# EmreAdabag/osqp

Hardware: AMD Instinct MI355X
Metric: ADMM iters/sec (single QP) (higher is better)
Workload: dtype f64; 1 GPU; config2 random sparse QP n=10000 m=20000 nnzA=200000 nnzPtriu=59985, one step = osqp_update_rho(0.1) + cold-started osqp_solve; adaptive_rho_interval=100, status=solved, graph_launches=4775, resident_gave_up=0, resident_slow_waits=0, parallelism=replicas x1 (a single QP does not shard)

## Files before the change

include/osqp_amd_engine.h:

```cpp
#ifndef OSQP_AMD_ENGINE_H
#define OSQP_AMD_ENGINE_H

#include "osqp_amd_types.h"

#ifdef __cplusplus
extern "C" {
#endif

#define HIPENG_OK            0
#define HIPENG_ERR_NO_DEVICE (-101)
#define HIPENG_ERR_HIP       (-102)
#define HIPENG_ERR_ARG       (-103)
#define HIPENG_ERR_ALLOC     (-104)

typedef struct hipeng hipeng;

typedef struct {
  c_float sigma;
  c_float alpha;
  c_float pcg_eps_rel;
  c_float pcg_eps_abs;
  c_int   pcg_max_iter;
  c_int   no_restart;
} hipeng_params;
// ... 50 lines not shown
int hipeng_certificates(hipeng *e, c_float eps_dx, int unscaled, hipeng_scalars *inout);
int hipeng_download(hipeng *e, c_float *x, c_float *y, c_float *z, c_float *dx,
                    c_float *dy, int dy_projected);
int hipeng_get_stats(hipeng *e, hipeng_stats *st);
int hipeng_reset_stats(hipeng *e);
int hipeng_sync(hipeng *e);

int hipeng_kkt_solve(hipeng *e, c_float *b);
int hipeng_kkt_solve_unrefined(hipeng *e, c_float *b);

int hipeng_spmv(hipeng *e, int which, const c_float *x, c_float *y);
int hipeng_spmv_dev(hipeng *e, int which, const c_float *d_x, c_float *d_y);
int hipeng_time_kernel(hipeng *e, int which, int reps, double *usec);
int hipeng_kernel_bytes(hipeng *e, int which, double *bytes);
int hipeng_is_split(hipeng *e);
int hipeng_pcg_layout(hipeng *e, long long out[16]);
int hipeng_row_eliminated(hipeng *e, c_int i);
c_int hipeng_elim_count(hipeng *e);
int hipeng_elim_peek(hipeng *e, int which, c_float *out);
int hipeng_resident_info(hipeng *e, long long out[16]);
int hipeng_resident_trips(hipeng *e, long long out[8]);
int hipeng_resident_plan(const csc *P, const csc *A, int nwg, long long stats[8], int *Kptr, int *Kcol, int *kdst, long long cap,
                         unsigned short *rowpos, unsigned short *slotcol, int *wg4);
long long hipeng_resident_plan_lists(const csc *P, const csc *A, int nwg, int *Kcp, int *Kcm, int *Kca, long long cap);
int hipeng_form_k_info(hipeng *e, long long out[4]);
long long hipeng_resident_dump(hipeng *e, int *row, int *col, double *val, long long cap);

int hipeng_dense_invert_selftest(int n, const double *A, double *Ainv, double *ms);
int hipeng_dense_invert_route(int n, const double *A, double *Ainv, int route, int gemm);
int hipeng_dense_switches(int out[2]);
int hipeng_dense_gemm_selftest(int kernel, int M, int N, int K, const double *T, int ldt, const double *B, int ldb, const double *w,
                               double *C, int ldc, double alpha, double beta, int sr0, int sr1, int sc0, int sc1, int lower, int kmode, int ksl);

int hipeng_switch_row(int index, const char **name, int *kind, char *def_text, int def_cap, int *unset_distinct, const char **what);
int hipeng_switch_values(double *out, int rows);

typedef struct hipsens hipsens;
int hipsens_create(hipsens **out, c_int n, c_int m, c_int nnzP, c_int nnzA, int device);
void hipsens_destroy(hipsens *s);
int hipsens_set_point(hipsens *s, hipeng *pe, const c_float *x, const c_float *yact, const c_int *act,
                      const c_float *D, const c_float *E, c_float c);
int hipsens_grad(hipsens *s, hipeng *pe, const csc *P, const csc *A, const c_float *rx, const c_float *rnu,
                 c_float *dPx, c_float *dAx);
int hipsens_tan_rhs(hipsens *s, hipeng *pe, const csc *P, const csc *A, c_int ndir, const c_float *dq, const c_float *dl,
                    const c_float *du, const c_float *dPx, const c_float *dAx, c_float *g);

// ... 15 lines not shown
```

osqp_amd/csrc/engine.hip:

```cpp
#include <hip/hip_runtime.h>
#include <cstdio>
#include <new>
#include <cstdlib>
#include <cstring>
#include <cstddef>
#include <climits>
#include <limits>
#include <cmath>
#include <vector>
#include <map>
#include <algorithm>
#include <mutex>
#include <condition_variable>
#include <thread>
#include <atomic>
#include <chrono>
#include "../../include/osqp_amd_engine.h"

#define TB 256
#define MAX_CHUNK 2048
#define LONG_ROW 512
#define HUGE_ROW 8192
#define MAX_PARTS 1024
#define MAX_HUGE_FOLD 4
// ... 1017 lines not shown
    __syncthreads();
  }
  for (int bi = c.A.nwave + blockIdx.x; bi < c.A.nblk; bi += gridDim.x) {
    const double zt = huge_row_sum(c, bi, red);
    if (threadIdx.x == 0) row_update(c.A.blk[bi].r0, zt);
    __syncthreads();
  }
  TLK_AT(8, 0); TLK_LAST(1);
  TLK_FLUSH(c, 110, 9);
}


#define RES_TB 512
#define RES_PT (RES_TB - 64)
#define RES_MAXROWS 61
#define RES_MAXN (RES_MAXROWS * 256)
#define RES_MAXPAD 16384
#define RES_MAXLD (RES_MAXPAD / 2 / RES_TB)
#define RES_WAIT_TICKS 2000000LL
#define RES_SLOW_TICKS 5000LL
#define AUX_SC1 16
#define AUX_VOL ((int)0x80000000)
#define RES_DBG 16
#define RES_PRED_WINDOW 16
#define RES_FSTRIDE 32
#define RES_GSTRIDE 16
typedef unsigned int u32x4 __attribute__((ext_vector_type(4)));
typedef unsigned int u32x2 __attribute__((ext_vector_type(2)));
struct ResWG { int r0, nr, cnt, pos; };
struct ResCtx {
  int nwg, E, npad;
  int npw;
  const unsigned short *rowpos;
  int pipe;
  int predict;
  double pred_margin;
  int u0_direct;
  int inject;
  const ResWG *wg;
  const int *ppos;
  double *val;
  const unsigned short *col;
  const unsigned char *rowl;
  const int *krp, *kcj, *kps, *kdst;
  const unsigned long long *brk;
  const unsigned short *slot0;
  const unsigned short *segrow;
  double *ubuf;
  unsigned *flags;
  int *dbg;
  double *sbuf;
  double *r0pos;
  const int *kcp, *kcm, *kca;
};

static __device__ __forceinline__ __amdgpu_buffer_rsrc_t res_rsrc(const void *p, size_t bytes) {
  return __builtin_amdgcn_make_buffer_rsrc(const_cast<void *>(p), 0, (int)bytes, 0x00020000);
}

__device__ __forceinline__ int res_spin_check(State *st, long long &t0, int &late) {
// ... 147 lines not shown
      }
#pragma unroll
      for (int q = 0; q < 4; ++q)
        if (eb + q * 64 + lane < e1) {
          const bool gone = c.nelim && (igone || c.erow[j[q]] >= 0);
          rc.val[dst[q]] = gone ? (j[q] == i ? 1.0 : 0.0) : v[q];
        }
    }
  }
}

template <int E>
__global__ void __launch_bounds__(RES_TB) k_pcg_resident(Ctx c, ResCtx rc) {
  extern __shared__ __attribute__((aligned(16))) double rlds[];
  State *st = c.st;
  TL_MARK(c, 5);
  const int s_stalled = st->stalled, s_run = st->run, s_fail = st->res_fail;
  const unsigned ep0 = st->res_epoch;
  const int s_pipe_off = st->res_pipe_off, s_pred_off = st->res_pred_off, s_admm_done = st->admm_done;
  const Params prm = *c.prm;
  const ResWG w = rc.wg[blockIdx.x];
  if ((s_stalled != 0) | (s_run == 0) | (s_fail != 0)) return;
  double *uv = rlds;
  double *seg = uv + rc.npad;
  double *sc = seg + RES_TB + RES_MAXROWS;
  double *sval = sc + 8;
#ifdef OSQP_AMD_TIMELINE
  long long *tls = reinterpret_cast<long long *>(sval + 768);
#define RTL(k) do { if (blockIdx.x == 0 && threadIdx.x == 0 && nx >= 1 && nx <= 64) tls[(nx - 1) * 5 + (k)] = wall_clock64(); } while (0)
  long long *wtl = tls + 5 * 64;
#define WTL(k) do { if (blockIdx.x == 0 && (threadIdx.x & 63) == 0 && (nx == 8 || nx == 1)) wtl[(nx == 1 ? 40 : 0) + (k) * 8 + (threadIdx.x >> 6)] = wall_clock64(); } while (0)
  if (blockIdx.x == 0 && threadIdx.x == 0) wtl[80] = wall_clock64();
#else
#define RTL(k) do { } while (0)
#define WTL(k) do { } while (0)
#endif
  const int g = blockIdx.x, t = threadIdx.x, lane = t & 63, wv = t >> 6;
  const int nwg = rc.nwg, npad = rc.npad;
  const bool sabotage = rc.inject > 0 && g == rc.nwg - 1 && s_admm_done + 1 == rc.inject;
  bool pipe = rc.pipe && !s_pipe_off && !prm.no_restart;
  bool predict = pipe && rc.predict && !s_pred_off;
  const bool prod = wv != 0;
  const int tt = t - 64;
  double kv[E]; unsigned short kc[E];
#pragma unroll
  for (int k = 0; k < E; ++k) { kv[k] = 0.0; kc[k] = 0; }
  unsigned long long brk = 0ull;
  int slot0 = 0;
  const bool u0_direct = rc.u0_direct != 0;
  u32x4 u0v[RES_MAXLD];
  auto u0_issue = [&]() __attribute__((always_inline)) {
    const __amdgpu_buffer_rsrc_t ru = res_rsrc(c.u0pos, (size_t)npad * 8);
#pragma unroll
    for (int q = 0; q < RES_MAXLD; ++q) u0v[q] = __builtin_amdgcn_raw_buffer_load_b128(ru, (q * RES_TB + t) * 16, 0, 0);
  };
  if (prod) {
    if (u0_direct) u0_issue();
#pragma unroll
    for (int k = 0; k < E; ++k) {
      const size_t idx = ((size_t)g * E + k) * RES_PT + tt;
      kv[k] = rc.val[idx]; kc[k] = rc.col[idx];
    }
    brk = rc.brk[(size_t)g * RES_PT + tt];
    slot0 = rc.slot0[(size_t)g * RES_PT + tt];
  }
  int sr0 = 0, sr1 = 0;
  int ppos[4] = {0, 0, 0, 0};
  constexpr int NPL = MAX_PARTS / 64;
  static_assert(NPL == 16 && NPL * 64 == MAX_PARTS, "k_pcg_resident: a lane of wavefront 0 holds MAX_PARTS / 64 partials of each start-up sum");
  double own_r = 0.0, own_u = 0.0, own_x = 0.0, own_mi = 0.0;
  if (!prod) {
    const int gm = c.gridM;
    double pr[NPL], pb[NPL];
#pragma unroll
    for (int q = 0; q < NPL; ++q) { const int i = min(lane + 64 * q, gm - 1); pr[q] = c.part_rr[i]; pb[q] = c.part_bb[i]; }
#pragma unroll
    for (int q = 0; q < 4; ++q) ppos[q] = rc.ppos[min(lane + 64 * q, nwg - 1)];
    const int jc = min(w.r0 + lane, c.n - 1), pc = min(w.pos + lane, npad - 1);
    const bool rpos = rc.r0pos != nullptr;
    const double *rsrc = rpos ? rc.r0pos : c.init_r, *usrc = rpos ? c.u0pos : c.init_z;
    own_r = rsrc[rpos ? (size_t)pc : (size_t)jc * c.init_stride]; own_u = usrc[rpos ? pc : jc]; own_x = c.vx[jc]; own_mi = c.minv[jc];
    sr0 = rc.segrow[(size_t)g * (RES_MAXROWS + 1) + min(lane, RES_MAXROWS)]; sr1 = rc.segrow[(size_t)g * (RES_MAXROWS + 1) + min(lane + 1, RES_MAXROWS)];
    double rr0 = 0.0, bb = 0.0;
#pragma unroll
    for (int q = 0; q < NPL; ++q) { const bool in = lane + 64 * q < gm; rr0 += in ? pr[q] : 0.0; bb += in ? pb[q] : 0.0; }
    rr0 = wave_sum(rr0); bb = wave_sum(bb);
    const double tl2 = fmax(prm.eps_rel * prm.eps_rel * bb, prm.eps_abs * prm.eps_abs);
    if (lane == 0) { sc[3] = 0.0; sc[5] = tl2; sc[6] = rr0 <= tl2 ? 1.0 : 0.0; }
    if (u0_direct) u0_issue();
  }
  const bool own = wv == 0 && lane < w.nr;
  const int j = w.r0 + lane;
  double rs_rest[11] = {0, 0, 0, 0, 0, 0, 0, 0, 0, 0, 0};
#define RES_ROWSTATE(i) (*((i) < E ? &kv[(i) < E ? (i) : 0] : &rs_rest[i]))
  double &r_ = RES_ROWSTATE(0), &u_ = RES_ROWSTATE(1), &w_ = RES_ROWSTATE(2), &p_ = RES_ROWSTATE(3), &s_ = RES_ROWSTATE(4), &x_ = RES_ROWSTATE(5);
  double &mi = RES_ROWSTATE(6), &x0_ = RES_ROWSTATE(7), &r0_ = RES_ROWSTATE(8);
  double &z_ = RES_ROWSTATE(9), &q_ = RES_ROWSTATE(10);
#undef RES_ROWSTATE
  if (own) { r_ = own_r; u_ = own_u; x_ = own_x; mi = own_mi; x0_ = own_x; r0_ = own_r; }
  else { sr0 = 0; sr1 = 0; }
  if (u0_direct) {
    const int half = npad >> 1;
#pragma unroll
    for (int q = 0; q < RES_MAXLD; ++q) {
      const int i2 = q * RES_TB + t;
      if (i2 < half) { uv[2 * i2] = __hiloint2double((int)u0v[q].y, (int)u0v[q].x); uv[2 * i2 + 1] = __hiloint2double((int)u0v[q].w, (int)u0v[q].z); }
    }
  }
  __syncthreads();
  const double tol2 = sc[5];
  if (sc[6] != 0.0) {
    if (g == 0 && t == 0) { st->done = 1; st->tol2 = tol2; }
    return;
  }
  int nx = 0;
  unsigned tag = ep0;
  int par = 0;

  auto vec_exchange = [&](double val, bool ride) __attribute__((always_inline)) -> bool {
    double e0 = 0.0, e1 = 0.0, e2 = 0.0;
    ++nx; tag = ep0 + (unsigned)nx; par = (int)(tag & 1u);
    if (sabotage && nx == 3) return false;
    RTL(0);
    const __amdgpu_buffer_rsrc_t rs = res_rsrc(rc.ubuf + (size_t)par * npad, (size_t)npad * 8);
    if (wv == 0) {
      if (lane < w.nr) {
        u32x2 d; d.x = (unsigned)__double2loint(val); d.y = (unsigned)__double2hiint(val);
        __builtin_amdgcn_raw_buffer_store_b64(d, rs, (w.pos + lane) * 8, 0, AUX_SC1);
      }
      if (ride) { e0 = wave_sum(own ? r_ * u_ : 0.0); e1 = wave_sum(own ? w_ * u_ : 0.0); e2 = wave_sum(own ? r_ * r_ : 0.0); }
      if (lane < 3) {
        const double v = lane == 0 ? e0 : (lane == 1 ? e1 : e2);
        u32x2 d; d.x = (unsigned)__double2loint(v); d.y = (unsigned)__double2hiint(v);
        __builtin_amdgcn_raw_buffer_store_b64(d, rs, (w.pos + w.nr + lane) * 8, 0, AUX_SC1);
      }
      asm volatile("s_waitcnt vmcnt(0)" ::: "memory");
      if (lane == 0) __hip_atomic_store(rc.flags + (size_t)g * RES_FSTRIDE, tag, __ATOMIC_RELAXED, __HIP_MEMORY_SCOPE_AGENT);
    }
    if (wv < rc.npw) {
      const int o = t;
// ... 14 lines not shown
        if (verdict) {
          const unsigned long long miss = __ballot(pend);
          const int fl = miss ? (int)__ffsll((long long)miss) - 1 : 0;
          const unsigned sv = (unsigned)__builtin_amdgcn_readlane((int)seen, fl);
          if (lane == 0) { res_note(st, rc.dbg, g, verdict, 1, nx, miss ? 64 * wv + fl : -1, sv, t0, rounds, 0); sc[3] = 1.0; }
          gave = true;
          break;
        }
        if (rounds == 16u) { const unsigned long long ms = __ballot(pend); miss16 = ms ? 64 * wv + (int)__ffsll((long long)ms) - 1 : -1; }
        if ((rounds & 63u) == 0 && wv == 0 && lane == 0) {
          __hip_atomic_store(rc.flags + (size_t)g * RES_FSTRIDE, tag, __ATOMIC_RELAXED, __HIP_MEMORY_SCOPE_AGENT);
          atomicAdd(&st->res_repub, 1);
        }
        if ((rounds & 255u) == 0) __builtin_amdgcn_fence(__ATOMIC_ACQUIRE, "agent");
        __builtin_amdgcn_s_sleep(1);
      }
      if (rounds >= 16u && lane == 0 && !gave) res_slow_note(st, t0, nx, g, miss16, 1);
    }
    __builtin_amdgcn_fence(__ATOMIC_ACQUIRE, "wavefront");
    __syncthreads();
    RTL(1);
    if (sc[3] != 0.0) return false;
    {
      const int half = npad >> 1;
      u32x4 v[RES_MAXLD];
#pragma unroll
      for (int q = 0; q < RES_MAXLD; ++q) { const int i2 = q * RES_TB + t; if (i2 < half) v[q] = __builtin_amdgcn_raw_buffer_load_b128(rs, i2 * 16, 0, AUX_SC1); }
#pragma unroll
      for (int q = 0; q < RES_MAXLD; ++q) {
        const int i2 = q * RES_TB + t;
        if (i2 < half) { uv[2 * i2] = __hiloint2double((int)v[q].y, (int)v[q].x); uv[2 * i2 + 1] = __hiloint2double((int)v[q].w, (int)v[q].z); }
      }
    }
    __syncthreads();
    RTL(2);
    return true;
  };
  auto products_issue = [&]() __attribute__((always_inline)) {
    if (prod) {
      double s = 0.0; int slot = slot0;
      constexpr int H = (E + 1) / 2;
#pragma unroll
      for (int h = 0; h < 2; ++h) {
        double xv[H];
#pragma unroll
        for (int k = 0; k < H; ++k) if (h * H + k < E) xv[k] = uv[kc[h * H + k]];
#pragma unroll
        for (int k = 0; k < H; ++k)
          if (h * H + k < E) {
            s += kv[h * H + k] * xv[k];
            if ((brk >> (h * H + k)) & 1ull) { seg[slot++] = s; s = 0.0; }
          }
      }
    }
  };
  auto products_finish = [&]() __attribute__((always_inline)) -> double {
    __syncthreads();
    RTL(3);
    double a = 0.0;
    if (own)
      for (int q0 = sr0; q0 < sr1; q0 += 16) {
        double sv[16];
#pragma unroll
        for (int q = 0; q < 16; ++q) sv[q] = seg[min(q0 + q, sr1 - 1)];
#pragma unroll
        for (int q = 0; q < 16; ++q) a += q0 + q < sr1 ? sv[q] : 0.0;
      }
    return a;
  };
  auto scal_exchange = [&](double pg, double pd, double prr) __attribute__((always_inline)) -> bool {
    unsigned long long *gb = reinterpret_cast<unsigned long long *>(rc.sbuf) + (size_t)par * nwg * RES_GSTRIDE;
    if (wv == 0) {
      pg = wave_sum(pg); pd = wave_sum(pd); prr = wave_sum(prr);
      if (lane < 6) {
// ... 1081 lines not shown
constexpr int SW_UNSET = -1;
struct Switches {
  int resident, resident_min_n, resident_all_cus, resident_nwg, resident_banks, resident_pipe, resident_predict;
  double resident_predict_margin;
  int resident_inject, resident_u0, resident_fine, resident_blocks, init_resident_stores, form_k_lists;
  double form_k_list_mb;
  int setup_threads, block_direct, block_coupled_max, block_fin_dots, block_plain;
  int dense_p, dense_direct, dense_small, dense_symv, dense_one_gather, dense_chol, dense_gemm_lds;
  int elim, hfold, split, chunk, fin_grid, fused_check;
  double extrap;
  int extrap_sched[2];
  int khead, graph_segs, trace;
  char trace_maps[PATH_MAX];
};
struct SwRow { const char *name; SwKind kind; size_t field; double def, def2; SwRange range; double lo, hi; bool unset_distinct; const char *what; };
#define SW(field) offsetof(Switches, field)
#define SW_NAME(x) "OSQP_AMD_" x
constexpr double SW_INF = std::numeric_limits<double>::infinity(), SW_TINY = std::numeric_limits<double>::denorm_min();
static const SwRow SW_TABLE[] = {
  {SW_NAME("RESIDENT"),                    SW_FLAG,     SW(resident),                 1, 0,    SW_ANY,    0, 0,           false, "0: never a one-launch form (resident PCG, block-resident PCG, block-direct solve)"},
  {SW_NAME("RESIDENT_MIN_N"),              SW_INT,      SW(resident_min_n),           256, 0,  SW_ANY,    0, 0,           false, "smallest n that takes the resident PCG"},
  {SW_NAME("RESIDENT_ALL_CUS"),            SW_FLAG,     SW(resident_all_cus),         0, 0,    SW_ANY,    0, 0,           false, "1: a resident grid may take every CU (default: one per XCD stays free)"},
  {SW_NAME("RESIDENT_NWG"),                SW_INT,      SW(resident_nwg),             0, 0,    SW_ANY,    0, 0,           false, "> 0: at least this many workgroups per resident launch, at most the plan's CUs (0: sized to the problem)"},
  {SW_NAME("RESIDENT_BANKS"),              SW_FLAG,     SW(resident_banks),           1, 0,    SW_ANY,    0, 0,           false, "0: a thread's entries of K in row order instead of spread over the LDS bank pairs"},
  {SW_NAME("RESIDENT_PIPE"),               SW_FLAG,     SW(resident_pipe),            1, 0,    SW_ANY,    0, 0,           false, "0: Chronopoulos-Gear recurrences only, never the pipelined ones"},
  {SW_NAME("RESIDENT_PREDICT"),            SW_FLAG,     SW(resident_predict),         1, 0,    SW_ANY,    0, 0,           false, "0: no predicted last trip in the pipelined phase"},
  {SW_NAME("RESIDENT_PREDICT_MARGIN"),     SW_DOUBLE,   SW(resident_predict_margin),  1.0, 0,  SW_IGNORE, SW_TINY, SW_INF, false, "last trip predicted at |r|^2 <= margin x tol^2; taken only if > 0"},
  {SW_NAME("RESIDENT_INJECT"),             SW_INT,      SW(resident_inject),          0, 0,    SW_ANY,    0, 0,           false, "test hook: the resident launch of ADMM iteration k gives up"},
  {SW_NAME("RESIDENT_U0"),                 SW_FLAG,     SW(resident_u0),              1, 0,    SW_ANY,    0, 0,           false, "0: exchange the first vector instead of reading it from memory"},
  {SW_NAME("RESIDENT_FINE"),               SW_INT,      SW(resident_fine),            2, 0,    SW_ANY,    0, 0,           false, "polled words in uncached (2), fine-grained (1) or ordinary (0) device memory"},
  {SW_NAME("RESIDENT_BLOCKS"),             SW_FLAG,     SW(resident_blocks),          1, 0,    SW_ANY,    0, 0,           false, "0: neither block form"},
  {SW_NAME("INIT_RESIDENT_STORES"),        SW_FLAG,     SW(init_resident_stores),     1, 0,    SW_ANY,    0, 0,           false, "0: k_pcg_init of the resident graphs also stores r0 and u0 where the launch-per-step kernels want them"},
  {SW_NAME("FORM_K_LISTS"),                SW_FLAG,     SW(form_k_lists),             1, 0,    SW_ANY,    0, 0,           false, "0: k_form_K (merge on the device) instead of k_form_K_lists"},
  {SW_NAME("FORM_K_LIST_MB"),              SW_DOUBLE,   SW(form_k_list_mb),           128.0, 0, SW_CLAMP, 0.0, 1e6,       false, "budget of the contribution lists in MiB"},
  {SW_NAME("SETUP_THREADS"),               SW_INT,      SW(setup_threads),            0, 0,    SW_CLAMP,  1, 64,          true,  "host threads of the resident set-up (unset: min(8, cores))"},
  {SW_NAME("BLOCK_DIRECT"),                SW_FLAG,     SW(block_direct),             1, 0,    SW_ANY,    0, 0,           false, "0: the block-resident PCG instead of the block-direct solve"},
  {SW_NAME("BLOCK_COUPLED_MAX"),           SW_INT,      SW(block_coupled_max),        CPL_MAX, 0, SW_CLAMP, 0, CPL_MAX,   false, "most coupling rows of A the block-direct solve carries as its low-rank term"},
  {SW_NAME("BLOCK_FIN_DOTS"),              SW_FLAG,     SW(block_fin_dots),           1, 0,    SW_ANY,    0, 0,           false, "0: a k_huge_dot launch per iteration even where the block-direct kernels could leave the partials"},
  {SW_NAME("BLOCK_PLAIN"),                 SW_FLAG,     SW(block_plain),              0, 0,    SW_ANY,    0, 0,           false, "1: block-direct solve on the right-hand side with the low-rank rows' terms split off"},
  {SW_NAME("DENSE_P"),                     SW_FLAG,     SW(dense_p),                  1, 0,    SW_ANY,    0, 0,           false, "0: no kernel path of their own for dense diagonal blocks of P"},
  {SW_NAME("DENSE_DIRECT"),                SW_INT,      SW(dense_direct),             1, 0,    SW_ANY,    0, 0,           false, "dense-direct solve: 0 never, 1 where it pays, 2 whenever it fits"},
  {SW_NAME("DENSE_SMALL"),                 SW_INT,      SW(dense_small),              1024, 0, SW_CLAMP,  0, INT_MAX,     false, "most dense unknowns that take the dense-direct solve ahead of the resident PCG (0: none)"},
  {SW_NAME("DENSE_SYMV"),                  SW_FLAG,     SW(dense_symv),               0, 0,    SW_ANY,    0, 0,           true,  "dense-direct solve from the inverse's lower tiles (1) or all its entries (0) (unset: tiles from 2048 unknowns up)"},
  {SW_NAME("DENSE_ONE_GATHER"),            SW_FLAG,     SW(dense_one_gather),         1, 0,    SW_ANY,    0, 0,           false, "0: dense-direct engines gather vb and vx separately in k_pcg_init"},
  {SW_NAME("DENSE_CHOL"),                  SW_FLAG,     SW(dense_chol),               0, 0,    SW_ANY,    0, 0,           true,  "1: blocked Cholesky inversion at once (unset: the caller's default -- 0 in an engine's refresh, 1 in hipeng_dense_invert_selftest)"},
  {SW_NAME("DENSE_GEMM_LDS"),              SW_FLAG,     SW(dense_gemm_lds),           1, 0,    SW_ANY,    0, 0,           false, "0: the dense-direct GEMM kernel that feeds the MFMAs from global memory"},
  {SW_NAME("ELIM"),                        SW_FLAG,     SW(elim),                     1, 0,    SW_ANY,    0, 0,           false, "0: no slack-like variable is eliminated from the linear system"},
// ... 386 lines not shown
        hipLaunchKernelGGL(k_cpl_dot, dim3(e->bd.kc), dim3(TB), 0, e->stream, e->c, e->bd, (const double *)e->bd.t, e->bd.cs, 1, 1, 0ll, 0ll, 1);
        hipLaunchKernelGGL(k_cpl_solve, dim3((e->bd.kc + TB / 64 - 1) / (TB / 64)), dim3(TB), 0, e->stream, e->c, e->bd);
        hipLaunchKernelGGL(k_blk_apply_back, dim3(gb), dim3(TB), 0, e->stream, e->c, e->bd);
      } else hipLaunchKernelGGL(k_blk_finish, dim3(std::max(1, std::min(256, (e->n + TB - 1) / TB))), dim3(TB), 0, e->stream, e->c, e->bd);
      return;
    case FORM_DENSE_DIRECT: launch_dense_direct(e); return;
  }
}

template <class F>
static void parallel_chunks(const Switches &sw, int count, int min_chunk, F fn) {
  int T = sw.setup_threads != SW_UNSET ? sw.setup_threads : (int)std::min<unsigned>(8u, std::max(1u, std::thread::hardware_concurrency()));
  T = std::min(T, std::max(1, count / min_chunk));
  if (T <= 1) { fn(0, count, 0, 1); return; }
  std::vector<std::thread> th;
  for (int k = 0; k < T; k++) th.emplace_back([=, &fn] { fn((int)((long long)count * k / T), (int)((long long)count * (k + 1) / T), k, T); });
  for (auto &t : th) t.join();
}

#define RES_NO(why) do { if (e->sw.trace) fprintf(stderr, "[osqp_amd] resident PCG not used: %s\n", why); return 0; } while (0)
struct ResPlanOut {
  bool ok = false; int nwg = 0, E = 0, npad = 0; long long nnzK = 0;
  std::vector<ResWG> wg; std::vector<int> Kptr, Kcol, kdst; std::vector<unsigned short> rowpos, col; std::vector<unsigned long long> brk;
  bool lists = false; std::vector<int> Kcp, Kcm, Kca;
};
static int build_resident(hipeng *e, int plan_nwg = 0, ResPlanOut *po = nullptr) {
  const int n = e->n;
  if (!e->sw.resident) RES_NO("OSQP_AMD_RESIDENT=0");
  if (n < e->sw.resident_min_n || n > RES_MAXN) RES_NO("n outside [OSQP_AMD_RESIDENT_MIN_N, 15616]");
  if (!e->hrows.empty() || e->A.nwave < (int)e->A.blk.size()) RES_NO("A has rows of 8192 or more entries");
  int nwg = plan_nwg < 0 ? -plan_nwg : plan_nwg;
  const bool fixed_grid = po && plan_nwg > 0;
  if (!po) {
    hipDeviceProp_t prop;
    HIPCHK(hipGetDeviceProperties(&prop, e->device));
    nwg = std::min(256, prop.multiProcessorCount) - 8;
    if (e->sw.resident_all_cus) nwg += 8;
    e->res_cus = nwg;
    if (prop.sharedMemPerBlock < 64 * 1024) RES_NO("too little LDS");
  }
  if (nwg <= 0 || nwg > 256 || (long long)nwg * RES_MAXROWS < n) RES_NO("too few CUs");
  const HostMat &M = e->M, &A = e->A;
  const auto tb0 = std::chrono::steady_clock::now();
  for (int i = 0; i < n; i++)
    for (int k = M.split[i] + 1; k < M.rowptr[i + 1]; k++) if (M.col[k] <= M.col[k - 1]) RES_NO("a column of A is not sorted by row (or repeats one)");
  const size_t cap_total = (size_t)nwg * RES_PT * 64;
// ... 115 lines not shown
    while (lo < hi) { const long long mid = (lo + hi) / 2; if (packs(mid) <= nwg) hi = mid; else lo = mid + 1; }
    C = lo;
    if (fixed_grid) { E = 0; for (int cand : RES_E_LIST) if ((long long)cand * RES_PT >= C) { E = cand; break; } if (!E) RES_NO("a row block of K exceeds 448 x 64 entries"); }
  }
  std::vector<ResWG> wg(nwg, ResWG{n, 0, 0, 0});
  {
    int g = 0, rows = 0; long long cnt = 0; wg[0].r0 = 0;
    for (int i = 0; i < n; i++) {
      const int len = Kptr[i + 1] - Kptr[i];
      if (rows > 0 && (cnt + len > C || rows == RES_MAXROWS)) { wg[g].nr = rows; wg[g].cnt = (int)cnt; g++; wg[g].r0 = i; cnt = 0; rows = 0; }
      cnt += len; rows++;
    }
    wg[g].nr = rows; wg[g].cnt = (int)cnt;
  }
  std::vector<unsigned short> rowpos(n, 0);
  int npad = 0;
  for (int g = 0; g < nwg; g++) {
    wg[g].pos = npad;
    for (int r = 0; r < wg[g].nr; r++) rowpos[wg[g].r0 + r] = (unsigned short)(npad + r);
    npad += ((wg[g].nr + 3 + 15) / 16) * 16;
  }
  if (npad > RES_MAXPAD) RES_NO("the exchanged vector (rows padded to whole lines) exceeds 16384 doubles");
  const size_t slots = (size_t)nwg * E * RES_PT;
  const bool bank_sched = e->sw.resident_banks != 0;
  std::vector<unsigned short> col(slots, 0), slot0((size_t)nwg * RES_PT, 0), segrow((size_t)nwg * (RES_MAXROWS + 1), 0);
  std::vector<unsigned char> rowl(slots, 0);
  std::vector<int> kdst((size_t)nnzK, 0);
  std::vector<unsigned long long> brk((size_t)nwg * RES_PT, 0ull);
  std::atomic<int> seg_over{0};
  parallel_chunks(e->sw, nwg, 4, [&](int g_lo, int g_hi, int, int) {
  for (int g = g_lo; g < g_hi; g++) {
    const ResWG &w = wg[g];
    if (w.nr == 0) continue;
    const int base = Kptr[w.r0];
    std::vector<int> rowof(w.cnt);
    for (int r = 0; r < w.nr; r++)
      for (int q = Kptr[w.r0 + r] - base; q < Kptr[w.r0 + r + 1] - base; q++) rowof[q] = r;
    std::vector<int> ord((size_t)RES_PT * E, -1);
    for (int le = 0; le < w.cnt; le++) ord[le] = le;
    if (bank_sched)
    for (int wq = 0; wq < RES_PT / 64; wq++) {
      int cntb[64][32];
      for (int k = 0; k < E; k++) for (int b = 0; b < 32; b++) cntb[k][b] = 0;
      bool freec[64];
      for (int l = 0; l < 64; l++) {
        const int t = wq * 64 + l, a = t * E;
        freec[l] = a + E <= w.cnt && rowof[a] == rowof[a + E - 1];
        if (!freec[l]) for (int k = 0; k < E && a + k < w.cnt; k++) cntb[k][rowpos[Kcol[base + a + k]] & 31]++;
      }
      for (int k = 0; k < E; k++)
        for (int l = 0; l < 64; l++) {
          if (!freec[l]) continue;
          const int a = (wq * 64 + l) * E;
          int best = k, bc = 1 << 30;
          for (int q = k; q < E; q++) { const int c = cntb[k][rowpos[Kcol[base + ord[a + q]]] & 31]; if (c < bc) { bc = c; best = q; } }
          std::swap(ord[a + k], ord[a + best]);
          cntb[k][rowpos[Kcol[base + ord[a + k]]] & 31]++;
        }
    }
    int nseg = 0, next_row = 0;
    for (int t = 0; t < RES_PT; t++) {
      slot0[(size_t)g * RES_PT + t] = (unsigned short)nseg;
      unsigned long long b = 0;
      for (int k = 0; k < E; k++) {
        if (t * E + k >= w.cnt) break;
        const int le = ord[t * E + k];
        const size_t sl = ((size_t)g * E + k) * RES_PT + t;
        col[sl] = rowpos[Kcol[base + le]]; rowl[sl] = (unsigned char)rowof[le]; kdst[base + le] = (int)sl;
        while (next_row <= rowof[le]) segrow[(size_t)g * (RES_MAXROWS + 1) + next_row++] = (unsigned short)nseg;
        const bool last = k == E - 1 || t * E + k + 1 >= w.cnt || rowof[ord[t * E + k + 1]] != rowof[le];
        if (last) { b |= 1ull << k; nseg++; }
      }
      brk[(size_t)g * RES_PT + t] = b;
    }
    for (int r = next_row; r <= RES_MAXROWS; r++) segrow[(size_t)g * (RES_MAXROWS + 1) + r] = (unsigned short)nseg;
    if (nseg > RES_TB + RES_MAXROWS) seg_over = 1;
  }
  });
  if (seg_over.load()) return 0;
  const auto tb2 = std::chrono::steady_clock::now();
  if (po) {
    po->ok = true; po->nwg = nwg; po->E = E; po->npad = npad; po->nnzK = nnzK;
    po->wg = wg; po->Kptr = Kptr; po->Kcol = Kcol; po->kdst = kdst; po->rowpos = rowpos; po->col = col; po->brk = brk;
    po->lists = fk_lists; po->Kcp = Kcp; po->Kcm = Kcm; po->Kca = Kca;
    return 0;
  }
  ResCtx rc{};
  rc.nwg = nwg; rc.E = E; rc.npad = npad;
  rc.npw = (nwg + 63) / 64;
  rc.pipe = e->sw.resident_pipe;
  rc.predict = e->sw.resident_predict; rc.pred_margin = e->sw.resident_predict_margin;
  rc.u0_direct = e->sw.resident_u0;
  rc.inject = e->sw.resident_inject;
  unsigned short *d_rowpos = nullptr;
  std::vector<int> ppos(wg.size());
  for (size_t o = 0; o < wg.size(); o++) ppos[o] = wg[o].pos + wg[o].nr;
  int *d_ppos = nullptr;
  ResWG *d_wg = nullptr; unsigned short *d_col = nullptr, *d_slot0 = nullptr, *d_segrow = nullptr; unsigned char *d_rowl = nullptr;
  int *d_krp = nullptr, *d_kcj = nullptr, *d_kps = nullptr, *d_kdst = nullptr; unsigned long long *d_brk = nullptr;
  if (dev_alloc(e, &d_wg, wg.size()) || dev_alloc(e, &d_ppos, ppos.size()) || dev_alloc(e, &rc.val, slots) || dev_alloc(e, &d_col, slots) || dev_alloc(e, &d_rowl, slots) ||
      dev_alloc(e, &d_krp, Kptr.size()) || dev_alloc(e, &d_kcj, Kcol.size()) || dev_alloc(e, &d_kps, Kps.size()) || dev_alloc(e, &d_kdst, kdst.size()) ||
      dev_alloc(e, &d_brk, brk.size()) || dev_alloc(e, &d_slot0, slot0.size()) ||
      dev_alloc(e, &d_segrow, segrow.size()) || dev_alloc(e, &d_rowpos, rowpos.size()) || dev_alloc(e, &rc.ubuf, (size_t)2 * rc.npad) ||
      dev_alloc_polled(e, &rc.flags, (size_t)nwg * RES_FSTRIDE) || dev_alloc(e, &rc.dbg, (size_t)nwg * RES_DBG) || dev_alloc_polled(e, &rc.sbuf, (size_t)2 * nwg * RES_GSTRIDE)) return HIPENG_ERR_HIP;
#define UP(dst, src) HIPCHK(hipMemcpyAsync(dst, (src).data(), (src).size() * sizeof((src)[0]), hipMemcpyHostToDevice, e->stream))
  if (fk_lists) {
    int *d_kcp = nullptr, *d_kcm = nullptr, *d_kca = nullptr;
    if (dev_alloc(e, &d_kcp, Kcp.size()) || dev_alloc(e, &d_kcm, Kcm.size()) || dev_alloc(e, &d_kca, Kca.size())) return HIPENG_ERR_HIP;
    UP(d_kcp, Kcp); UP(d_kcm, Kcm); UP(d_kca, Kca);
    rc.kcp = d_kcp; rc.kcm = d_kcm; rc.kca = d_kca;
  }
  e->fk_lists = fk_lists; e->fk_terms = fk_terms; e->fk_bytes = fk_lists ? fk_bytes(nnzK) : 0; e->fk_budget = fk_budget;
  UP(d_wg, wg); UP(d_ppos, ppos); UP(d_rowpos, rowpos); UP(d_col, col); UP(d_rowl, rowl); UP(d_krp, Kptr); UP(d_kcj, Kcol); UP(d_kps, Kps); UP(d_kdst, kdst); UP(d_brk, brk); UP(d_slot0, slot0); UP(d_segrow, segrow);
#undef UP
  HIPCHK(hipStreamSynchronize(e->stream));
  {
    double *d_u0pos = nullptr;
    if (dev_alloc(e, &d_u0pos, (size_t)rc.npad)) return HIPENG_ERR_HIP;
    e->c.u0map = d_rowpos; e->c.u0pos = d_u0pos;
    rc.r0pos = nullptr;
    if (e->sw.init_resident_stores && dev_alloc(e, &rc.r0pos, (size_t)rc.npad)) return HIPENG_ERR_HIP;
  }
  rc.wg = d_wg; rc.ppos = d_ppos; rc.rowpos = d_rowpos; rc.col = d_col; rc.rowl = d_rowl; rc.krp = d_krp; rc.kcj = d_kcj; rc.kps = d_kps; rc.kdst = d_kdst; rc.brk = d_brk; rc.slot0 = d_slot0; rc.segrow = d_segrow;
  e->rc = rc;
  e->res_lds = ((size_t)rc.npad + RES_TB + RES_MAXROWS + 3 + 16 + 768 + 5 * 64 + 96) * sizeof(double);
  int rcode = 0;
  switch (E) {
    case 8: rcode = res_set_lds<8>(e->res_lds); break;   case 16: rcode = res_set_lds<16>(e->res_lds); break;
    case 20: rcode = res_set_lds<20>(e->res_lds); break; case 24: rcode = res_set_lds<24>(e->res_lds); break;
    case 32: rcode = res_set_lds<32>(e->res_lds); break; case 48: rcode = res_set_lds<48>(e->res_lds); break;
    default: rcode = res_set_lds<64>(e->res_lds); break;
  }
  if (rcode) RES_NO("the launch's LDS request was refused");
  e->res_nnz = nnzK;
  e->form = FORM_RESIDENT; e->res_use = true;
  if (e->sw.trace) {
    const auto tb3 = std::chrono::steady_clock::now();
    auto ms = [](std::chrono::steady_clock::time_point a, std::chrono::steady_clock::time_point b) { return std::chrono::duration<double, std::milli>(b - a).count(); };
    fprintf(stderr, "[osqp_amd] resident PCG: nnz(K)=%lld, %d workgroups x %d threads x %d entries, %zu B LDS; host: pattern %.0f ms, layout %.0f ms, upload %.0f ms\n",
            nnzK, nwg, RES_TB, E, e->res_lds, ms(tb0, tb1), ms(tb1, tb2), ms(tb2, tb3));
  }
  return 0;
}


static bool blocks_eligible(hipeng *e) {
  if (e->dP_blks.empty()) return false;
  int next = 0;
// ... 1079 lines not shown
extern "C" int hipeng_resident_plan(const csc *P, const csc *A, int nwg, long long stats[8], int *Kptr, int *Kcol, int *kdst, long long cap,
                                    unsigned short *rowpos, unsigned short *slotcol, int *wg4) {
  if (!P || !A || !stats || P->n > 0x7ffffff0LL || A->m > 0x7ffffff0LL) return HIPENG_ERR_ARG;
  hipeng tmp;
  tmp.n = (int)P->n; tmp.m = (int)A->m;
  build_A(&tmp, A); build_M(&tmp, P, A); build_dense(&tmp, P);
  ResPlanOut po;
  const int rc = build_resident(&tmp, nwg, &po);
  for (int k = 0; k < 8; k++) stats[k] = 0;
  if (rc) return rc;
  stats[0] = po.ok; stats[7] = RES_PT;
  if (!po.ok) return 0;
  stats[1] = po.E; stats[2] = po.npad; stats[3] = po.nnzK;
  for (const ResWG &w : po.wg) { if (w.nr) stats[4]++; stats[5] = std::max<long long>(stats[5], w.nr); stats[6] = std::max<long long>(stats[6], w.cnt); }
  if (Kptr) std::copy(po.Kptr.begin(), po.Kptr.end(), Kptr);
  if (po.nnzK <= cap) { if (Kcol) std::copy(po.Kcol.begin(), po.Kcol.end(), Kcol); if (kdst) std::copy(po.kdst.begin(), po.kdst.end(), kdst); }
  else if (Kcol || kdst) return HIPENG_ERR_ARG;
  if (rowpos) std::copy(po.rowpos.begin(), po.rowpos.end(), rowpos);
  if (slotcol) std::copy(po.col.begin(), po.col.end(), slotcol);
  if (wg4) for (size_t g = 0; g < po.wg.size(); g++) { wg4[4 * g] = po.wg[g].r0; wg4[4 * g + 1] = po.wg[g].nr; wg4[4 * g + 2] = po.wg[g].cnt; wg4[4 * g + 3] = po.wg[g].pos; }
  return 0;
}

extern "C" long long hipeng_resident_plan_lists(const csc *P, const csc *A, int nwg, int *Kcp, int *Kcm, int *Kca, long long cap) {
  if (!P || !A || P->n > 0x7ffffff0LL || A->m > 0x7ffffff0LL) return HIPENG_ERR_ARG;
  hipeng tmp;
  tmp.n = (int)P->n; tmp.m = (int)A->m;
  build_A(&tmp, A); build_M(&tmp, P, A); build_dense(&tmp, P);
  ResPlanOut po;
  if (const int rc = build_resident(&tmp, nwg, &po)) return rc;
  if (!po.ok) return -1;
  if (!po.lists) return -2;
  const long long terms = (long long)po.Kcm.size();
  if (Kcp) std::copy(po.Kcp.begin(), po.Kcp.end(), Kcp);
  if (terms <= cap) { if (Kcm) std::copy(po.Kcm.begin(), po.Kcm.end(), Kcm); if (Kca) std::copy(po.Kca.begin(), po.Kca.end(), Kca); }
  else if (Kcm || Kca) return HIPENG_ERR_ARG;
  return terms;
}

extern "C" int hipeng_switch_row(int index, const char **name, int *kind, char *def_text, int def_cap, int *unset_distinct, const char **what) {
  if (index < 0 || index >= SW_COUNT) return SW_COUNT;
  const SwRow &r = SW_TABLE[index];
  if (name) *name = r.name;
  if (kind) *kind = r.kind;
  if (unset_distinct) *unset_distinct = r.unset_distinct;
  if (what) *what = r.what;
// ... 134 lines not shown
```

Baseline: 8609 ADMM iters/s.

## Group resident PCG product chunks by class and add branch-free single-row wavefront path

In the resident PCG kernel, each thread's chunk of K entries is now placed through a permutation that groups single-row chunks, mixed chunks and empty chunks together. A wavefront whose chunks all lie in one row takes a plain dot-product path with no per-entry segment-break branching. The LDS bank scheduler is also rewritten to work per 32-lane half-wave with iterative swap passes that lower the worst bank conflict count. The LDS vector copy loop drops its per-element bound check in favour of a whole-row count. The cost is an extra indirection load per thread, slightly more LDS padding and a longer host-side plan build.

```diff
diff --git a/include/osqp_amd_engine.h b/include/osqp_amd_engine.h
--- a/include/osqp_amd_engine.h
+++ b/include/osqp_amd_engine.h
@@ -96,6 +96,8 @@
 int hipeng_resident_trips(hipeng *e, long long out[8]);
 int hipeng_resident_plan(const csc *P, const csc *A, int nwg, long long stats[8], int *Kptr, int *Kcol, int *kdst, long long cap,
                          unsigned short *rowpos, unsigned short *slotcol, int *wg4);
+int hipeng_resident_plan_products(const csc *P, const csc *A, int nwg, unsigned short *place, unsigned long long *brk,
+                                  unsigned short *slot0, unsigned short *segrow, unsigned char *rowl);
 long long hipeng_resident_plan_lists(const csc *P, const csc *A, int nwg, int *Kcp, int *Kcm, int *Kca, long long cap);
 int hipeng_form_k_info(hipeng *e, long long out[4]);
 long long hipeng_resident_dump(hipeng *e, int *row, int *col, double *val, long long cap);
diff --git a/osqp_amd/csrc/engine.hip b/osqp_amd/csrc/engine.hip
--- a/osqp_amd/csrc/engine.hip
+++ b/osqp_amd/csrc/engine.hip
@@ -1063,6 +1063,7 @@
 #define AUX_SC1 16
 #define AUX_VOL ((int)0x80000000)
 #define RES_DBG 16
+#define RES_DEAL_PASSES 8
 #define RES_PRED_WINDOW 16
 #define RES_FSTRIDE 32
 #define RES_GSTRIDE 16
@@ -1077,6 +1078,8 @@
   int predict;
   double pred_margin;
   int u0_direct;
+  int plain;
+  const unsigned short *chunk;
   int inject;
   const ResWG *wg;
   const int *ppos;
@@ -1270,7 +1273,8 @@
   const ResWG w = rc.wg[blockIdx.x];
   if ((s_stalled != 0) | (s_run == 0) | (s_fail != 0)) return;
   double *uv = rlds;
-  double *seg = uv + rc.npad;
+  const int nrow = (rc.npad + 2 * RES_TB - 1) / (2 * RES_TB);
+  double *seg = uv + nrow * 2 * RES_TB;
   double *sc = seg + RES_TB + RES_MAXROWS;
   double *sval = sc + 8;
 #ifdef OSQP_AMD_TIMELINE
@@ -1303,14 +1307,15 @@
     for (int q = 0; q < RES_MAXLD; ++q) u0v[q] = __builtin_amdgcn_raw_buffer_load_b128(ru, (q * RES_TB + t) * 16, 0, 0);
   };
   if (prod) {
+    const int ch = rc.chunk[(size_t)g * RES_PT + tt];
     if (u0_direct) u0_issue();
 #pragma unroll
     for (int k = 0; k < E; ++k) {
-      const size_t idx = ((size_t)g * E + k) * RES_PT + tt;
+      const size_t idx = ((size_t)g * E + k) * RES_PT + ch;
       kv[k] = rc.val[idx]; kc[k] = rc.col[idx];
     }
-    brk = rc.brk[(size_t)g * RES_PT + tt];
-    slot0 = rc.slot0[(size_t)g * RES_PT + tt];
+    brk = rc.brk[(size_t)g * RES_PT + ch];
+    slot0 = rc.slot0[(size_t)g * RES_PT + ch];
   }
   int sr0 = 0, sr1 = 0;
   int ppos[4] = {0, 0, 0, 0};
@@ -1348,11 +1353,10 @@
   if (own) { r_ = own_r; u_ = own_u; x_ = own_x; mi = own_mi; x0_ = own_x; r0_ = own_r; }
   else { sr0 = 0; sr1 = 0; }
   if (u0_direct) {
-    const int half = npad >> 1;
 #pragma unroll
     for (int q = 0; q < RES_MAXLD; ++q) {
       const int i2 = q * RES_TB + t;
-      if (i2 < half) { uv[2 * i2] = __hiloint2double((int)u0v[q].y, (int)u0v[q].x); uv[2 * i2 + 1] = __hiloint2double((int)u0v[q].w, (int)u0v[q].z); }
+      if (q == 0 || q < nrow) { uv[2 * i2] = __hiloint2double((int)u0v[q].y, (int)u0v[q].x); uv[2 * i2 + 1] = __hiloint2double((int)u0v[q].w, (int)u0v[q].z); }
     }
   }
   __syncthreads();
@@ -1364,6 +1368,7 @@
   int nx = 0;
   unsigned tag = ep0;
   int par = 0;
+  const bool wplain = prod && rc.plain && __ballot(brk != 0ull && brk != (1ull << (E - 1))) == 0ull;
 
   auto vec_exchange = [&](double val, bool ride) __attribute__((always_inline)) -> bool {
     double e0 = 0.0, e1 = 0.0, e2 = 0.0;
@@ -1424,14 +1429,15 @@
     RTL(1);
     if (sc[3] != 0.0) return false;
     {
-      const int half = npad >> 1;
       u32x4 v[RES_MAXLD];
 #pragma unroll
-      for (int q = 0; q < RES_MAXLD; ++q) { const int i2 = q * RES_TB + t; if (i2 < half) v[q] = __builtin_amdgcn_raw_buffer_load_b128(rs, i2 * 16, 0, AUX_SC1); }
+      for (int q = 0; q < RES_MAXLD; ++q) v[q] = __builtin_amdgcn_raw_buffer_load_b128(rs, (q * RES_TB + t) * 16, 0, AUX_SC1);
+      int nr = nrow;
+      asm volatile("" : "+s"(nr));
 #pragma unroll
       for (int q = 0; q < RES_MAXLD; ++q) {
         const int i2 = q * RES_TB + t;
-        if (i2 < half) { uv[2 * i2] = __hiloint2double((int)v[q].y, (int)v[q].x); uv[2 * i2 + 1] = __hiloint2double((int)v[q].w, (int)v[q].z); }
+        if (q == 0 || q < nr) { uv[2 * i2] = __hiloint2double((int)v[q].y, (int)v[q].x); uv[2 * i2 + 1] = __hiloint2double((int)v[q].w, (int)v[q].z); }
       }
     }
     __syncthreads();
@@ -1439,7 +1445,22 @@
     return true;
   };
   auto products_issue = [&]() __attribute__((always_inline)) {
-    if (prod) {
+    if (wplain) {
+      double s = 0.0;
+      constexpr int H = (E + 1) / 2;
+#pragma unroll
+      for (int h = 0; h < 2; ++h) {
+        double xv[H];
+#pragma unroll
+        for (int k = 0; k < H; ++k) if (h * H + k < E) xv[k] = uv[kc[h * H + k]];
+        asm volatile("" ::: "memory");
+#pragma unroll
+        for (int k = 0; k < H; ++k) if (h * H + k < E) s += kv[h * H + k] * xv[k];
+      }
+      if (brk != 0ull) seg[slot0] = s;
+    } else if (prod) {
+      unsigned long long bk = brk;
+      asm volatile("" : "+v"(bk));
       double s = 0.0; int slot = slot0;
       constexpr int H = (E + 1) / 2;
 #pragma unroll
@@ -1451,7 +1472,7 @@
         for (int k = 0; k < H; ++k)
           if (h * H + k < E) {
             s += kv[h * H + k] * xv[k];
-            if ((brk >> (h * H + k)) & 1ull) { seg[slot++] = s; s = 0.0; }
+            if ((bk >> (h * H + k)) & 1ull) { seg[slot++] = s; s = 0.0; }
           }
       }
     }
@@ -2579,7 +2600,7 @@
   {SW_NAME("RESIDENT_MIN_N"),              SW_INT,      SW(resident_min_n),           256, 0,  SW_ANY,    0, 0,           false, "smallest n that takes the resident PCG"},
   {SW_NAME("RESIDENT_ALL_CUS"),            SW_FLAG,     SW(resident_all_cus),         0, 0,    SW_ANY,    0, 0,           false, "1: a resident grid may take every CU (default: one per XCD stays free)"},
   {SW_NAME("RESIDENT_NWG"),                SW_INT,      SW(resident_nwg),             0, 0,    SW_ANY,    0, 0,           false, "> 0: at least this many workgroups per resident launch, at most the plan's CUs (0: sized to the problem)"},
-  {SW_NAME("RESIDENT_BANKS"),              SW_FLAG,     SW(resident_banks),           1, 0,    SW_ANY,    0, 0,           false, "0: a thread's entries of K in row order instead of spread over the LDS bank pairs"},
+  {SW_NAME("RESIDENT_BANKS"),              SW_INT,      SW(resident_banks),           1, 0,    SW_ANY,    0, 0,           false, "0: a thread's entries of K in row order instead of spread over the LDS bank pairs; 2, 3: as 0, 1 and every product wavefront on the general path"},
   {SW_NAME("RESIDENT_PIPE"),               SW_FLAG,     SW(resident_pipe),            1, 0,    SW_ANY,    0, 0,           false, "0: Chronopoulos-Gear recurrences only, never the pipelined ones"},
   {SW_NAME("RESIDENT_PREDICT"),            SW_FLAG,     SW(resident_predict),         1, 0,    SW_ANY,    0, 0,           false, "0: no predicted last trip in the pipelined phase"},
   {SW_NAME("RESIDENT_PREDICT_MARGIN"),     SW_DOUBLE,   SW(resident_predict_margin),  1.0, 0,  SW_IGNORE, SW_TINY, SW_INF, false, "last trip predicted at |r|^2 <= margin x tol^2; taken only if > 0"},
@@ -3012,6 +3033,7 @@
 struct ResPlanOut {
   bool ok = false; int nwg = 0, E = 0, npad = 0; long long nnzK = 0;
   std::vector<ResWG> wg; std::vector<int> Kptr, Kcol, kdst; std::vector<unsigned short> rowpos, col; std::vector<unsigned long long> brk;
+  std::vector<unsigned short> place, slot0, segrow; std::vector<unsigned char> rowl;
   bool lists = false; std::vector<int> Kcp, Kcm, Kca;
 };
 static int build_resident(hipeng *e, int plan_nwg = 0, ResPlanOut *po = nullptr) {
@@ -3173,11 +3195,14 @@
   }
   if (npad > RES_MAXPAD) RES_NO("the exchanged vector (rows padded to whole lines) exceeds 16384 doubles");
   const size_t slots = (size_t)nwg * E * RES_PT;
-  const bool bank_sched = e->sw.resident_banks != 0;
+  const bool bank_sched = (e->sw.resident_banks & 1) != 0;
   std::vector<unsigned short> col(slots, 0), slot0((size_t)nwg * RES_PT, 0), segrow((size_t)nwg * (RES_MAXROWS + 1), 0);
   std::vector<unsigned char> rowl(slots, 0);
   std::vector<int> kdst((size_t)nnzK, 0);
   std::vector<unsigned long long> brk((size_t)nwg * RES_PT, 0ull);
+  std::vector<unsigned short> place((size_t)nwg * RES_PT, 0);
+  for (size_t q = 0; q < place.size(); q++) place[q] = (unsigned short)(q % RES_PT);
+  std::vector<unsigned short> chunk_of = place;
   std::atomic<int> seg_over{0};
   parallel_chunks(e->sw, nwg, 4, [&](int g_lo, int g_hi, int, int) {
   for (int g = g_lo; g < g_hi; g++) {
@@ -3187,39 +3212,69 @@
     std::vector<int> rowof(w.cnt);
     for (int r = 0; r < w.nr; r++)
       for (int q = Kptr[w.r0 + r] - base; q < Kptr[w.r0 + r + 1] - base; q++) rowof[q] = r;
+    auto chunk_class = [&](int c) { const int a = c * E; return a >= w.cnt ? 2 : (a + E <= w.cnt && rowof[a] == rowof[a + E - 1] ? 1 : 0); };
+    unsigned short *pl = &place[(size_t)g * RES_PT];
+    int chunk_at[RES_PT];
+    {
+      int p = 0;
+      for (int cl = 0; cl < 3; cl++)
+        for (int c = 0; c < RES_PT; c++) if (chunk_class(c) == cl) { pl[c] = (unsigned short)p; chunk_at[p++] = c; }
+    }
     std::vector<int> ord((size_t)RES_PT * E, -1);
     for (int le = 0; le < w.cnt; le++) ord[le] = le;
     if (bank_sched)
-    for (int wq = 0; wq < RES_PT / 64; wq++) {
-      int cntb[64][32];
+    for (int hq = 0; hq < RES_PT / 32; hq++) {
+      int cntb[64][32], worst[64];
       for (int k = 0; k < E; k++) for (int b = 0; b < 32; b++) cntb[k][b] = 0;
-      bool freec[64];
-      for (int l = 0; l < 64; l++) {
-        const int t = wq * 64 + l, a = t * E;
-        freec[l] = a + E <= w.cnt && rowof[a] == rowof[a + E - 1];
-        if (!freec[l]) for (int k = 0; k < E && a + k < w.cnt; k++) cntb[k][rowpos[Kcol[base + a + k]] & 31]++;
-      }
-      for (int k = 0; k < E; k++)
-        for (int l = 0; l < 64; l++) {
+      bool freec[32], any_free = false;
+      for (int l = 0; l < 32; l++) {
+        const int c = chunk_at[hq * 32 + l], a = c * E;
+        freec[l] = chunk_class(c) == 1;
+        any_free = any_free || freec[l];
+        for (int k = 0; k < E && a + k < w.cnt; k++) cntb[k][rowpos[Kcol[base + a + k]] & 31]++;
+      }
+      if (!any_free) continue;
+      for (int k = 0; k < E; k++) { worst[k] = 0; for (int b = 0; b < 32; b++) worst[k] = std::max(worst[k], cntb[k][b]); }
+      for (int pass = 0; pass < RES_DEAL_PASSES; pass++) {
+        bool moved = false;
+        for (int l = 0; l < 32; l++) {
           if (!freec[l]) continue;
-          const int a = (wq * 64 + l) * E;
-          int best = k, bc = 1 << 30;
-          for (int q = k; q < E; q++) { const int c = cntb[k][rowpos[Kcol[base + ord[a + q]]] & 31]; if (c < bc) { bc = c; best = q; } }
-          std::swap(ord[a + k], ord[a + best]);
-          cntb[k][rowpos[Kcol[base + ord[a + k]]] & 31]++;
+          const int a = chunk_at[hq * 32 + l] * E;
+          for (int k = 0; k < E; k++) {
+            int bk = rowpos[Kcol[base + ord[a + k]]] & 31;
+            if (cntb[k][bk] == 1) continue;
+            int best = -1, gain = 0;
+            for (int q = 0; q < E; q++) {
+              const int bq = rowpos[Kcol[base + ord[a + q]]] & 31;
+              if (q == k || bq == bk) continue;
+              if (cntb[k][bq] + 1 > worst[k] || cntb[q][bk] + 1 > worst[q]) continue;
+              const int d = (cntb[k][bk] - cntb[k][bq] - 1) + (cntb[q][bq] - cntb[q][bk] - 1);
+              if (d > gain) { gain = d; best = q; }
+            }
+            if (best < 0) continue;
+            const int bq = rowpos[Kcol[base + ord[a + best]]] & 31;
+            cntb[k][bk]--; cntb[k][bq]++; cntb[best][bq]--; cntb[best][bk]++;
+            std::swap(ord[a + k], ord[a + best]);
+            moved = true;
+          }
         }
+        if (!moved) break;
+        for (int k = 0; k < E; k++) { worst[k] = 0; for (int b = 0; b < 32; b++) worst[k] = std::max(worst[k], cntb[k][b]); }
+      }
     }
     int nseg = 0, next_row = 0;
-    for (int t = 0; t < RES_PT; t++) {
+    for (int c = 0; c < RES_PT; c++) {
+      const int t = c;
+      chunk_of[(size_t)g * RES_PT + pl[c]] = (unsigned short)c;
       slot0[(size_t)g * RES_PT + t] = (unsigned short)nseg;
       unsigned long long b = 0;
       for (int k = 0; k < E; k++) {
-        if (t * E + k >= w.cnt) break;
-        const int le = ord[t * E + k];
+        if (c * E + k >= w.cnt) break;
+        const int le = ord[c * E + k];
         const size_t sl = ((size_t)g * E + k) * RES_PT + t;
         col[sl] = rowpos[Kcol[base + le]]; rowl[sl] = (unsigned char)rowof[le]; kdst[base + le] = (int)sl;
         while (next_row <= rowof[le]) segrow[(size_t)g * (RES_MAXROWS + 1) + next_row++] = (unsigned short)nseg;
-        const bool last = k == E - 1 || t * E + k + 1 >= w.cnt || rowof[ord[t * E + k + 1]] != rowof[le];
+        const bool last = k == E - 1 || c * E + k + 1 >= w.cnt || rowof[ord[c * E + k + 1]] != rowof[le];
         if (last) { b |= 1ull << k; nseg++; }
       }
       brk[(size_t)g * RES_PT + t] = b;
@@ -3233,6 +3288,7 @@
   if (po) {
     po->ok = true; po->nwg = nwg; po->E = E; po->npad = npad; po->nnzK = nnzK;
     po->wg = wg; po->Kptr = Kptr; po->Kcol = Kcol; po->kdst = kdst; po->rowpos = rowpos; po->col = col; po->brk = brk;
+    po->place = place; po->slot0 = slot0; po->segrow = segrow; po->rowl = rowl;
     po->lists = fk_lists; po->Kcp = Kcp; po->Kcm = Kcm; po->Kca = Kca;
     return 0;
   }
@@ -3242,16 +3298,17 @@
   rc.pipe = e->sw.resident_pipe;
   rc.predict = e->sw.resident_predict; rc.pred_margin = e->sw.resident_predict_margin;
   rc.u0_direct = e->sw.resident_u0;
+  rc.plain = (e->sw.resident_banks & 2) == 0;
   rc.inject = e->sw.resident_inject;
   unsigned short *d_rowpos = nullptr;
   std::vector<int> ppos(wg.size());
   for (size_t o = 0; o < wg.size(); o++) ppos[o] = wg[o].pos + wg[o].nr;
   int *d_ppos = nullptr;
-  ResWG *d_wg = nullptr; unsigned short *d_col = nullptr, *d_slot0 = nullptr, *d_segrow = nullptr; unsigned char *d_rowl = nullptr;
+  ResWG *d_wg = nullptr; unsigned short *d_col = nullptr, *d_chunk = nullptr, *d_slot0 = nullptr, *d_segrow = nullptr; unsigned char *d_rowl = nullptr;
   int *d_krp = nullptr, *d_kcj = nullptr, *d_kps = nullptr, *d_kdst = nullptr; unsigned long long *d_brk = nullptr;
   if (dev_alloc(e, &d_wg, wg.size()) || dev_alloc(e, &d_ppos, ppos.size()) || dev_alloc(e, &rc.val, slots) || dev_alloc(e, &d_col, slots) || dev_alloc(e, &d_rowl, slots) ||
       dev_alloc(e, &d_krp, Kptr.size()) || dev_alloc(e, &d_kcj, Kcol.size()) || dev_alloc(e, &d_kps, Kps.size()) || dev_alloc(e, &d_kdst, kdst.size()) ||
-      dev_alloc(e, &d_brk, brk.size()) || dev_alloc(e, &d_slot0, slot0.size()) ||
+      dev_alloc(e, &d_brk, brk.size()) || dev_alloc(e, &d_slot0, slot0.size()) || dev_alloc(e, &d_chunk, chunk_of.size()) ||
       dev_alloc(e, &d_segrow, segrow.size()) || dev_alloc(e, &d_rowpos, rowpos.size()) || dev_alloc(e, &rc.ubuf, (size_t)2 * rc.npad) ||
       dev_alloc_polled(e, &rc.flags, (size_t)nwg * RES_FSTRIDE) || dev_alloc(e, &rc.dbg, (size_t)nwg * RES_DBG) || dev_alloc_polled(e, &rc.sbuf, (size_t)2 * nwg * RES_GSTRIDE)) return HIPENG_ERR_HIP;
 #define UP(dst, src) HIPCHK(hipMemcpyAsync(dst, (src).data(), (src).size() * sizeof((src)[0]), hipMemcpyHostToDevice, e->stream))
@@ -3262,7 +3319,7 @@
     rc.kcp = d_kcp; rc.kcm = d_kcm; rc.kca = d_kca;
   }
   e->fk_lists = fk_lists; e->fk_terms = fk_terms; e->fk_bytes = fk_lists ? fk_bytes(nnzK) : 0; e->fk_budget = fk_budget;
-  UP(d_wg, wg); UP(d_ppos, ppos); UP(d_rowpos, rowpos); UP(d_col, col); UP(d_rowl, rowl); UP(d_krp, Kptr); UP(d_kcj, Kcol); UP(d_kps, Kps); UP(d_kdst, kdst); UP(d_brk, brk); UP(d_slot0, slot0); UP(d_segrow, segrow);
+  UP(d_wg, wg); UP(d_ppos, ppos); UP(d_rowpos, rowpos); UP(d_col, col); UP(d_rowl, rowl); UP(d_krp, Kptr); UP(d_kcj, Kcol); UP(d_kps, Kps); UP(d_kdst, kdst); UP(d_brk, brk); UP(d_slot0, slot0); UP(d_chunk, chunk_of); UP(d_segrow, segrow);
 #undef UP
   HIPCHK(hipStreamSynchronize(e->stream));
   {
@@ -3272,9 +3329,9 @@
     rc.r0pos = nullptr;
     if (e->sw.init_resident_stores && dev_alloc(e, &rc.r0pos, (size_t)rc.npad)) return HIPENG_ERR_HIP;
   }
-  rc.wg = d_wg; rc.ppos = d_ppos; rc.rowpos = d_rowpos; rc.col = d_col; rc.rowl = d_rowl; rc.krp = d_krp; rc.kcj = d_kcj; rc.kps = d_kps; rc.kdst = d_kdst; rc.brk = d_brk; rc.slot0 = d_slot0; rc.segrow = d_segrow;
+  rc.wg = d_wg; rc.ppos = d_ppos; rc.rowpos = d_rowpos; rc.col = d_col; rc.rowl = d_rowl; rc.krp = d_krp; rc.kcj = d_kcj; rc.kps = d_kps; rc.kdst = d_kdst; rc.brk = d_brk; rc.slot0 = d_slot0; rc.chunk = d_chunk; rc.segrow = d_segrow;
   e->rc = rc;
-  e->res_lds = ((size_t)rc.npad + RES_TB + RES_MAXROWS + 3 + 16 + 768 + 5 * 64 + 96) * sizeof(double);
+  e->res_lds = ((size_t)(rc.npad + 2 * RES_TB - 1) / (2 * RES_TB) * (2 * RES_TB) + RES_TB + RES_MAXROWS + 3 + 16 + 768 + 5 * 64 + 96) * sizeof(double);
   int rcode = 0;
   switch (E) {
     case 8: rcode = res_set_lds<8>(e->res_lds); break;   case 16: rcode = res_set_lds<16>(e->res_lds); break;
@@ -4400,6 +4457,23 @@
   return 0;
 }
 
+extern "C" int hipeng_resident_plan_products(const csc *P, const csc *A, int nwg, unsigned short *place, unsigned long long *brk,
+                                             unsigned short *slot0, unsigned short *segrow, unsigned char *rowl) {
+  if (!P || !A || P->n > 0x7ffffff0LL || A->m > 0x7ffffff0LL) return HIPENG_ERR_ARG;
+  hipeng tmp;
+  tmp.n = (int)P->n; tmp.m = (int)A->m;
+  build_A(&tmp, A); build_M(&tmp, P, A); build_dense(&tmp, P);
+  ResPlanOut po;
+  if (const int rc = build_resident(&tmp, nwg, &po)) return rc;
+  if (!po.ok) return HIPENG_ERR_ARG;
+  if (place) std::copy(po.place.begin(), po.place.end(), place);
+  if (brk) std::copy(po.brk.begin(), po.brk.end(), brk);
+  if (slot0) std::copy(po.slot0.begin(), po.slot0.end(), slot0);
+  if (segrow) std::copy(po.segrow.begin(), po.segrow.end(), segrow);
+  if (rowl) std::copy(po.rowl.begin(), po.rowl.end(), rowl);
+  return 0;
+}
+
 extern "C" long long hipeng_resident_plan_lists(const csc *P, const csc *A, int nwg, int *Kcp, int *Kcm, int *Kca, long long cap) {
   if (!P || !A || P->n > 0x7ffffff0LL || A->m > 0x7ffffff0LL) return HIPENG_ERR_ARG;
   hipeng tmp;
```

After: 8661 ADMM iters/s, median of 6. About the same (+0.6%).
